# frozenreboot/rplidar_ros2_driver

Measured on AMD Instinct MI355X. Metric: Mpoints/s raw-scan->filtered PointCloud2, higher is better.
Workload: dtype u32/f32

## Files before the change

rplidar_ros2_driver_amd/csrc/rpl_device.hpp:

```cpp
#pragma once
#include <hip/hip_runtime.h>
#include <stdint.h>

#include "rplgpu.h"

namespace rpl {

constexpr int kBlock = 1024;
constexpr int kWaves = kBlock / 64;
constexpr int kIters = 32;
constexpr uint32_t kMaxN = 32768;
constexpr int kChunks = kIters * kWaves;
constexpr double kTwoPi = 6.283185307179586476925286766559;

struct Tables {
  const float *angle;
  const float *angle_inv;
  const float2 *cs;
  const float2 *cs_inv;
  const double *rcp;
  uint32_t *work_ctr;
  uint32_t n_cu;
  void *voxel_store;
  uint32_t voxel_store_wgs;
  uint32_t voxel_store_recs;
  unsigned long long *voxel_stats;
  unsigned long long *voxel_stats_host;
  int32_t voxel_split;
  const float *scan_t0;
  uint32_t *redo;
};

struct KParams {
  int32_t is_new_protocol;
  int32_t inverted;
  int32_t scan_processing;
  int32_t clip_enable;
  uint32_t q_min;
  float range_min;
  float range_max;
  float voxel_leaf;
  float ror_r2;
  uint32_t ror_k;
  double vox_scale;
  float vox_scale_f;
  int32_t vox_L;
  int32_t vox_bias;
  float inv_leaf;
  float leaf_s;
  float inv_leaf_s;
  uint32_t d_lo;
  uint32_t d_span;
  int32_t cell_range_safe;
  unsigned long long *dbg;
  uint32_t *cell_keys;
  int32_t fast_div;
  int32_t fast_d4000;
};

__device__ __forceinline__ uint32_t nd_q14(uint2 v) { return v.x & 0xFFFFu; }
// ... 114 lines not shown
```

rplidar_ros2_driver_amd/csrc/rpl_launch.hpp:

```cpp
#pragma once
#include <hip/hip_runtime.h>
#include <stdint.h>

#include "rplgpu.h"
#include "rplgpu_msg.h"
#include "rplgpu_comm.h"
#include "rpl_device.hpp"
#include "rpl_msg.hpp"

namespace rplmsg {
struct Prefix;
}

namespace rpl {

constexpr uint32_t kAscendUnsorted = 0x80000000u;
constexpr uint32_t kRorListedBit = 0x80000000u;
constexpr uint32_t kScanStatusBits =
    RPLGPU_SCAN_ALL_INVALID | RPLGPU_SCAN_CELL_RANGE | RPLGPU_SCAN_TABLE_FULL | RPLGPU_SCAN_OUT_TRUNCATED;
static_assert((kAscendUnsorted & kScanStatusBits) == 0, "internal ascend bit overlaps RPLGPU_SCAN_*");
static_assert((kRorListedBit & kScanStatusBits) == 0, "internal cloud bit overlaps RPLGPU_SCAN_*");
hipError_t launch_ascend(hipStream_t s, void *nodes, uint32_t n_stride, const uint32_t *n_per_scan,
                         uint32_t B, uint32_t *status, uint32_t *need_sort, bool defer_sort = false,
                         uint32_t *sort_stat = nullptr);
// ... 13 lines not shown
                              const Tables &T, const float *inc_table, const float *rinc_table,
                              bool fast, float *ranges, float *intens, uint32_t *beam_count,
                              uint32_t n_given = 0xFFFFFFFFu, const LsMsgOut *msg_out = nullptr);
hipError_t launch_validate_idx(hipStream_t s, const Tables &T, const float *inc_table,
                               const float *rinc_table, uint32_t max_count,
                               uint32_t *d_mismatches);
hipError_t launch_laserscan_raw(hipStream_t s, const void *nodes, uint32_t n_stride,
                                const uint32_t *n_per_scan, uint32_t B, const KParams &p,
                                float *ranges, float *intens, uint32_t *beam_count);
hipError_t launch_cloud(hipStream_t s, const void *nodes, uint32_t n_stride,
                        const uint32_t *n_per_scan, uint32_t B, const KParams &p, const Tables &T,
                        const uint32_t *keepmask, uint32_t mask_stride, float *xyzi,
                        uint32_t out_stride, uint32_t *n_points, uint32_t *status,
                        const float *motion = nullptr);
enum class ArenaForm : int { kXyzi = 0, kXyi = 1, kCells = 2 };
enum class RorMode : int { kNone = 0, kInside = 1, kListed = 2 };
struct VoxelLaunch {
  const void *nodes = nullptr;
  uint32_t n_stride = 0;
  const uint32_t *n_per_scan = nullptr;
  uint32_t B = 0;
  uint32_t group = 1;
  const float *motion = nullptr, *pose2d = nullptr;
  const uint32_t *keepmask = nullptr;
  uint32_t mask_stride = 0;
  RorMode ror = RorMode::kNone;
  float *xyzi = nullptr;
  uint32_t out_stride = 0;
  float *arena = nullptr;
  uint64_t arena_capacity = 0;
  uint64_t *arena_cursor = nullptr, *scan_start = nullptr;
  ArenaForm form = ArenaForm::kXyzi;
  uint32_t *n_points = nullptr, *status = nullptr;
};
hipError_t launch_cloud_voxel(hipStream_t s, const VoxelLaunch &v, const KParams &p, const Tables &T);
uint32_t voxel_max_workgroups(uint32_t n_cu);
inline uint64_t voxel_store_need(uint32_t group, uint32_t n_stride) {
  const uint64_t s = n_stride < kMaxN ? n_stride : kMaxN;
  return (uint64_t)(group ? group : 1u) * (s + 2u * ((s + 123u) / 124u) + 1u + 528u);
}
hipError_t launch_ror_mask(hipStream_t s, const void *nodes, uint32_t n_stride,
                           const uint32_t *n_per_scan, uint32_t B, const KParams &p,
                           const Tables &T, uint32_t *mask, uint32_t mask_stride,
                           bool listed = false, uint32_t group = 1);
hipError_t launch_validate_div(hipStream_t s, float d, float rd, uint32_t e_lo, uint32_t e_hi,
                               uint32_t *d_mismatches);
hipError_t launch_pack(hipStream_t s, const float *xyzi, uint32_t out_stride,
                       const uint32_t *n_points, uint32_t B, float *packed, uint64_t *offsets);

hipError_t launch_laserscan_to_cloud(hipStream_t s, const float *ranges, const float *intens,
                                     uint32_t n_stride, const uint32_t *beam_count, uint32_t B,
                                     const KParams &p, float *xyzi, uint32_t out_stride,
                                     uint32_t *n_points, uint32_t *status);

hipError_t launch_signal(hipStream_t s, uint32_t *flag, uint32_t seq);
hipError_t launch_stage_in(hipStream_t s, const void *src, void *dst, uint32_t n_words2);
hipError_t launch_pack_meta(hipStream_t s, const unsigned long long *cursor,
                            const unsigned long long *scan_start, const uint32_t *n_points,
                            uint32_t B, unsigned long long slot_points, uint32_t max_scans,
                            uint32_t *meta);
hipError_t launch_unpack_gathered(hipStream_t s, const float *points_all,
                                  unsigned long long slot_points, const uint32_t *meta_all,
                                  uint32_t meta_words, uint32_t world, uint32_t max_scans,
                                  float *packed, unsigned long long *total,
                                  unsigned long long *scan_start_all, uint32_t *n_points_all,
                                  uint32_t *status, uint32_t n_cu, bool xyi = false);
// ... 193 lines not shown
```

rplidar_ros2_driver_amd/csrc/rpl_voxel.hip:

```cpp
#include <algorithm>
#include <cstdlib>
#include <type_traits>

#include "rpl_device.hpp"
#include "rpl_launch.hpp"
#include "rpl_xf.hpp"

namespace rpl {

#ifndef RPL_VOXEL_THREADS
#define RPL_VOXEL_THREADS 1024
#endif
#ifndef RPL_VOXEL_WGS_PER_CU
#define RPL_VOXEL_WGS_PER_CU (RPL_VOXEL_THREADS == 512 ? 2 : 1)
#endif
constexpr int kVB = RPL_VOXEL_THREADS;
constexpr int kVW = kVB / 64;
constexpr int kVWG = RPL_VOXEL_WGS_PER_CU;
constexpr uint32_t kRecCap = kVWG == 2 ? 4096u : 7168u;
constexpr uint32_t kRecPerThread = kRecCap / kVB;
constexpr uint32_t kRowCap = kVWG == 2 ? 1024u : 2u * kVB;
constexpr uint32_t kRowsPerThread = kRowCap / kVB;
constexpr uint32_t kBucketCap = kRecCap + 3u * kRowCap;
constexpr uint32_t kEmptyKey = 0xFFFFFFFFu;
// ... 262 lines not shown
  return false;
}

template <int NS>
__device__ __forceinline__ void voxel_block_split(QueueSink &S,
                                                  const bool (&ok)[NS], const uint32_t (&key)[NS],
                                                  const uint32_t (&qx)[NS], const uint32_t (&qy)[NS],
                                                  const uint32_t (&ci)[NS]) {
#pragma unroll
  for (uint32_t cls = 0; cls < 2u; ++cls) {
    bool okc[NS];
    uint32_t keyc[NS], qxc[NS], qyc[NS], cic[NS];
#pragma unroll
    for (int j = 0; j < NS; ++j) {
      okc[j] = ok[j] && (((key[j] >> 16) ^ key[j]) & 1u) == cls;
      keyc[j] = key[j];
      qxc[j] = okc[j] ? qx[j] : 0u;
      qyc[j] = okc[j] ? qy[j] : 0u;
      cic[j] = okc[j] ? ci[j] : 0u;
    }
    voxel_block_pass<true, NS, kPassPlain>(S, okc, keyc, qxc, qyc, cic);
  }
}

__device__ __forceinline__ double run_sum_f64(uint32_t u) {
  double s = (double)u;
  if (u >= 0xF0000000u) s -= 4294967296.0;
  return s;
}

struct VoxelArena {
  float4 *base;
  unsigned long long *cursor;
  unsigned long long capacity;
  unsigned long long *scan_start;
  int xyi;
};
enum : int { kEmitLegacy = 0, kEmitArenaFirst = 1, kEmitCountOnly = 2, kEmitArenaKnown = 3, kEmitArenaTemp = 4 };

template <bool DBG>
struct PhaseClock {
  unsigned long long acc[8] = {0, 0, 0, 0, 0, 0, 0, 0}, mark = 0;
  __device__ __forceinline__ void start() {
    if (DBG) mark = clock64();
  }
  __device__ __forceinline__ void lap(int i) {
    if (DBG) {
      const unsigned long long now = clock64();
      acc[i] += now - mark;
      mark = now;
    }
  }
};

template <bool DBG, bool CELLS>
__device__ __forceinline__ uint32_t voxel_reduce(VoxelLds &L, const KParams &p,
                                                 float4 *__restrict__ out, uint32_t out_stride,
                                                 uint32_t b, uint32_t *ncell_out, int mode,
                                                 const VoxelArena &arena, bool normalised,
                                                 const float4 *out_buffer) {
  PhaseClock<DBG> pc;
  pc.start();
  auto flush_dbg = [&]() {
    if (DBG && p.dbg && threadIdx.x == 0) {
#pragma unroll
      for (int i = 1; i < 8; ++i) atomicAdd(&p.dbg[16 * b + i], pc.acc[i]);
// ... 511 lines not shown
                                                      unsigned long long *dbg_slot,
                                                      RorSide *rs = nullptr, uint32_t oob_off = 0u) {
  if constexpr (RORM == 1) {
    if (use_xf)
      voxel_stream<FAST_DIV, SAFE, SPLIT, false, true, false, true, AHEAD, true>(
          sink, p, cs, rsrc, blk0, blk_end, nullptr, 0u, sd.xf, q_min16, ibfe_off, ibfe_w, flags, nullptr, rs, oob_off);
    else if (q_min16)
      voxel_stream<FAST_DIV, SAFE, SPLIT, false, true, false, false, AHEAD, true>(
          sink, p, cs, rsrc, blk0, blk_end, nullptr, 0u, sd.xf, q_min16, ibfe_off, ibfe_w, flags, nullptr, rs, oob_off);
    else
      voxel_stream<FAST_DIV, SAFE, SPLIT, false, false, false, false, AHEAD, true>(
          sink, p, cs, rsrc, blk0, blk_end, nullptr, 0u, sd.xf, q_min16, ibfe_off, ibfe_w, flags, nullptr, rs, oob_off);
    return;
  }
#define RPL_VS(HQ, HM, XFB)                                                                         \
  voxel_stream<FAST_DIV, SAFE, SPLIT, DBG, HQ, HM, XFB, AHEAD>(sink, p, cs, rsrc, blk0, blk_end, \
                                                                     sd.ror_bits, mask_stride, sd.xf, \
                                                                     q_min16, ibfe_off, ibfe_w, flags, \
                                                                     dbg_slot)
  if constexpr (RORM == 2) {
    if (use_xf) RPL_VS(true, true, true);
    else RPL_VS(true, true, false);
    return;
  }
  if (use_xf) {
    if (sd.ror_bits) RPL_VS(true, true, true);
    else RPL_VS(true, false, true);
  } else if (sd.ror_bits) RPL_VS(true, true, false);
  else if (q_min16) RPL_VS(true, false, false);
  else RPL_VS(false, false, false);
#undef RPL_VS
}

template <bool DBG, int RORM = 0, bool CELLS = false, class FirstBand>
__device__ __forceinline__ void voxel_work_loop(VoxelLds &L, const KParams &p, const Tables &T,
                                                uint4 *__restrict__ G, float4 *__restrict__ xyzi,
                                                uint32_t out_stride, uint32_t *__restrict__ n_points,
                                                uint32_t *__restrict__ status, uint32_t B,
                                                uint32_t item0, const VoxelArena &arena,
                                                FirstBand &&first_band) {
  if (threadIdx.x < 256) L.rcp[threadIdx.x] = T.rcp[threadIdx.x];
  if constexpr (RORM == 2) B = min(B, (uint32_t)__builtin_amdgcn_readfirstlane((int)T.redo[0]));
  for (uint32_t bl = blockIdx.x; bl < B;) {
  const uint32_t b = RORM == 2 ? T.redo[4u + bl] : item0 + bl;
  bool abandoned = false;
  float4 *out = arena.base ? arena.base : xyzi + (size_t)b * out_stride;
  int emit_mode = arena.base ? kEmitArenaFirst : kEmitLegacy;
  unsigned long long arena_at = 0ull;

  if (threadIdx.x < 16) L.misc[threadIdx.x] = 0u;
  if (threadIdx.x == 0) {
    L.band_lo[0] = 0u;
    L.band_hi[0] = 0xFFFFFFFEu;
    L.misc[3] = 1u;
    L.tmp[28] = 0u;
    L.tmp[29] = 0u;
  }
  __syncthreads();

  uint32_t flags = 0;
  PhaseClock<DBG> pc;
  pc.start();

  bool first = true;
  bool leave_single_band_mode_early = false;
  bool from_store = false;
// ... 294 lines not shown
        float *dst = reinterpret_cast<float *>(arena.base) + 3u * (size_t)arena_at;
        for (uint32_t i = threadIdx.x; i < ncopy; i += kVB) {
          const float4 v = src[i];
          dst[3u * i] = v.x;
          dst[3u * i + 1u] = v.y;
          dst[3u * i + 2u] = v.w;
        }
      } else {
        float4 *dst = arena.base + arena_at;
        for (uint32_t i = threadIdx.x; i < ncopy; i += kVB) dst[i] = src[i];
      }
    }
  }
  if (DBG && p.dbg && threadIdx.x == 0) {
    atomicAdd(&p.dbg[16 * b], pc.acc[0]);
    atomicAdd(&p.dbg[16 * b + 2], pc.acc[2]);
  }

  if (flags) atomicOr(&L.misc[1], flags);
  __syncthreads();
  if (threadIdx.x == 0 && !abandoned) {
    const uint32_t total = L.misc[7];
    if (arena.base) {
      const unsigned long long room = arena_at >= arena.capacity ? 0ull : arena.capacity - arena_at;
      const uint32_t kept = (uint32_t)min((unsigned long long)total, room);
      arena.scan_start[b] = arena_at;
      n_points[b] = kept;
      if (status) status[b] = L.misc[1] | (kept < total ? RPLGPU_SCAN_OUT_TRUNCATED : 0u);
    } else {
      n_points[b] = min(total, out_stride);
      if (status) status[b] = L.misc[1] | ((total > out_stride) ? RPLGPU_SCAN_OUT_TRUNCATED : 0u);
    }
  }
  if (RORM != 2 && B <= gridDim.x) return;
  if (threadIdx.x == 0) L.tmp[31] = gridDim.x + atomicAdd(&T.work_ctr[0], 1u);
  __syncthreads();
  bl = L.tmp[31];
  __syncthreads();
  }
}

template <bool FAST_DIV, bool SAFE, bool DBG, bool SPLIT, int RORM = 0>
__global__ __launch_bounds__(kVB) __attribute__((amdgpu_waves_per_eu(kVB * kVWG / 256, kVB * kVWG / 256))) void k_cloud_voxel(
    const uint2 *__restrict__ nodes, uint32_t n_stride, const uint32_t *__restrict__ n_per_scan,
    KParams p, Tables T, const uint32_t *__restrict__ keepmask, uint32_t mask_stride,
    float4 *__restrict__ xyzi, uint32_t out_stride, uint32_t *__restrict__ n_points,
    uint32_t *__restrict__ status, uint32_t B, VoxelArena arena, uint4 *__restrict__ store,
    uint32_t group, uint32_t n_scans, const float *__restrict__ motion,
    const float *__restrict__ pose2d) {
  __shared__ VoxelLds L;
  uint4 *G = store + (size_t)blockIdx.x * 2u * T.voxel_store_recs;
  const float2 *cs = p.inverted ? T.cs_inv : T.cs;
  const uint32_t ishift = p.is_new_protocol ? 0u : 2u;
  const uint32_t ibfe_off = 16u + ishift, ibfe_w = 0xFFu >> ishift;
  const uint32_t q_min16 = p.clip_enable ? (min(p.q_min, 256u) << 16) : 0u;
  const bool use_xf = (group > 1u) || motion || pose2d;
  __shared__ RorSide Rs;
  auto phase_s = [&](uint32_t b, uint32_t, uint32_t &flags) -> bool {
    QueueSink sink{L, G};
    const uint32_t s_lo = b * group, s_hi = min(n_scans, s_lo + group);
    for (uint32_t sc = s_lo; sc < s_hi; ++sc) {
      const uint32_t n = (uint32_t)__builtin_amdgcn_readfirstlane(
          (int)min(n_per_scan[sc], min(n_stride, kMaxN)));
      const uint2 *scan = nodes + (size_t)sc * n_stride;
      const __amdgpu_buffer_rsrc_t scan_rsrc =
          __builtin_amdgcn_make_buffer_rsrc((void *)scan, 0, (int)(n * 8u), 0x00020000);
      const ScanSide sd = scan_side(sc, keepmask, mask_stride, motion, pose2d, T.scan_t0);
      const uint32_t blk0 = (uint32_t)__builtin_amdgcn_readfirstlane((int)wave_id());
      if constexpr (RORM == 1) {
        if (threadIdx.x == 0) { Rs.n_todo = 0u; Rs.n_todo2 = 0u; }
        __syncthreads();
        voxel_stream_dispatch<FAST_DIV, SAFE, SPLIT, false, RPL_VOXEL_AHEAD, 1>(
// ... 38 lines not shown
    bad += (div_by(0.0f, d, rd) != 0.0f);
    bad += (div_by(-0.0f, d, rd) != 0.0f);
  }
  if (bad) atomicAdd(mismatches, bad);
}

hipError_t launch_validate_div(hipStream_t s, float d, float rd, uint32_t e_lo, uint32_t e_hi,
                               uint32_t *d_mismatches) {
  hipLaunchKernelGGL(k_validate_div, dim3(256 * 16), dim3(256), 0, s, d, rd, e_lo, e_hi,
                     d_mismatches);
  return hipGetLastError();
}

uint32_t voxel_max_workgroups(uint32_t n_cu) { return (uint32_t)kVWG * (n_cu ? n_cu : 256u); }


hipError_t launch_cloud_voxel(hipStream_t s, const VoxelLaunch &v, const KParams &p, const Tables &T) {
  static_assert(sizeof(unsigned long long) == sizeof(uint64_t), "64-bit cursor");
  uint32_t B = v.B, group = v.group;
  const bool ror = v.ror != RorMode::kNone, listed = v.ror == RorMode::kListed;
  if (B == 0) return hipSuccess;
  if (ror && (!p.fast_div || !T.redo || p.dbg)) return hipErrorInvalidValue;
  if (listed && !v.keepmask) return hipErrorInvalidValue;
  if (v.form == ArenaForm::kCells && !ror && (p.dbg || !T.voxel_split)) return hipErrorInvalidValue;
  if (group == 0) group = 1;
  group = std::min(group, B);
  const uint32_t n_scans = B;
  B = (B + group - 1u) / group;
  if (!T.voxel_store || T.voxel_store_wgs == 0) return hipErrorInvalidValue;
  if (voxel_store_need(group, v.n_stride) > T.voxel_store_recs) return hipErrorInvalidValue;
  VoxelArena ar;
  ar.base = (float4 *)v.arena;
  ar.cursor = reinterpret_cast<unsigned long long *>(v.arena_cursor);
  ar.capacity = v.arena_capacity;
  ar.scan_start = reinterpret_cast<unsigned long long *>(v.scan_start);
  ar.xyi = v.arena ? (int)v.form : 0;
  if (kVWG == 2 && group > 1) return hipErrorInvalidValue;
  uint32_t grid = std::min<uint32_t>(std::min<uint32_t>(B, voxel_max_workgroups(T.n_cu)),
                                     T.voxel_store_wgs);
  if (const char *e = std::getenv("RPLGPU_VOXEL_GRID")) {
    const long g = std::atol(e);
    if (g > 0) grid = std::min<uint32_t>(grid, (uint32_t)g);
  }
  const bool with_stats = T.voxel_stats && T.voxel_stats_host && B >= 64u && !listed;
  Tables Tk = T;
  if (!with_stats) Tk.voxel_stats = nullptr;
  if (with_stats)
    if (hipError_t e = hipMemsetAsync(T.voxel_stats, 0, 16, s); e != hipSuccess) return e;
  if (grid < B || listed)
    if (hipError_t e = hipMemsetAsync(T.work_ctr, 0, 4, s); e != hipSuccess) return e;
#define RPL_LAUNCH_VOXEL(FD, SF, DB, SP)                                                          \
  hipLaunchKernelGGL((k_cloud_voxel<FD, SF, DB, SP>), dim3(grid), dim3(kVB), 0, s, (const uint2 *)v.nodes, \
                     v.n_stride, v.n_per_scan, p, Tk, v.keepmask, v.mask_stride, (float4 *)v.xyzi, v.out_stride, \
                     v.n_points, v.status, B, ar, (uint4 *)T.voxel_store, group, n_scans, v.motion, v.pose2d)
#define RPL_LAUNCH_VOXEL_SF(FD, DB, SP)                                                           \
  do {                                                                                             \
    if (p.cell_range_safe) RPL_LAUNCH_VOXEL(FD, true, DB, SP); else RPL_LAUNCH_VOXEL(FD, false, DB, SP); \
  } while (0)
#define RPL_LAUNCH_VOXEL_ROR(SF, SP, RM)                                                          \
  hipLaunchKernelGGL((k_cloud_voxel<true, SF, false, SP, RM>), dim3(grid), dim3(kVB), 0, s,         \
                     (const uint2 *)v.nodes, v.n_stride, v.n_per_scan, p, Tk, v.keepmask, v.mask_stride, \
                     (float4 *)v.xyzi, v.out_stride, v.n_points, v.status, B, ar, (uint4 *)T.voxel_store, \
                     group, n_scans, v.motion, v.pose2d)
#define RPL_LAUNCH_VOXEL_ROR_SF(SP, RM)                                                           \
  do {                                                                                             \
    if (p.cell_range_safe) RPL_LAUNCH_VOXEL_ROR(true, SP, RM); else RPL_LAUNCH_VOXEL_ROR(false, SP, RM); \
  } while (0)
  if (v.ror == RorMode::kInside) {
    if (T.voxel_split) RPL_LAUNCH_VOXEL_ROR_SF(true, 1); else RPL_LAUNCH_VOXEL_ROR_SF(false, 1);
  } else if (listed) {
    if (T.voxel_split) RPL_LAUNCH_VOXEL_ROR_SF(true, 2); else RPL_LAUNCH_VOXEL_ROR_SF(false, 2);
  } else
  if (p.dbg) {
    if (p.fast_div) RPL_LAUNCH_VOXEL_SF(true, true, false); else RPL_LAUNCH_VOXEL_SF(false, true, false);
  } else if (T.voxel_split) {
    if (p.fast_div) RPL_LAUNCH_VOXEL_SF(true, false, true); else RPL_LAUNCH_VOXEL_SF(false, false, true);
  } else {
    if (p.fast_div) RPL_LAUNCH_VOXEL_SF(true, false, false); else RPL_LAUNCH_VOXEL_SF(false, false, false);
  }
#undef RPL_LAUNCH_VOXEL_SF
#undef RPL_LAUNCH_VOXEL
#undef RPL_LAUNCH_VOXEL_ROR_SF
#undef RPL_LAUNCH_VOXEL_ROR
  if (with_stats) {
    if (hipError_t e = hipMemcpyAsync(T.voxel_stats_host, T.voxel_stats, 16, hipMemcpyDeviceToHost, s);
        e != hipSuccess)
      return e;
  }
  return hipGetLastError();
}

}
```

rplidar_ros2_driver_amd/csrc/rplgpu_api.hip:

```cpp
#include <hip/hip_runtime.h>
#include <dlfcn.h>

#include <algorithm>
#include <cmath>
#include <cstdio>
#include <cstdlib>
#include <cstring>
#include <limits>
#include <new>
#include <string>
#include <thread>
#include <vector>

#include "rplgpu.h"
#include "rplgpu_msg.h"
#include "rpl_launch.hpp"
#include "rpl_msg.hpp"
#include "rpl_comm_layout.hpp"
#include "rpl_cells.hpp"

struct VoxelBatchId {
  const void *nodes = nullptr;
  uint32_t n_stride = 0, B = 0, group = 0;
  bool operator==(const VoxelBatchId &o) const {
    return nodes == o.nodes && n_stride == o.n_stride && B == o.B && group == o.group;
  }
};

struct rplgpu_ctx {
  int device = -1;
  hipStream_t own_stream = nullptr;
  hipStream_t stream = nullptr;
  uint32_t max_n = 0, max_b = 0;
  float *d_angle = nullptr, *d_angle_inv = nullptr, *d_inc = nullptr, *d_rinc = nullptr;
  float2 *d_cs = nullptr, *d_cs_inv = nullptr;
  double *d_rcp = nullptr;
  unsigned char *h_pin = nullptr;
  unsigned char *d_pin = nullptr;
  bool zero_copy = true;
  bool spin_sync = true;
  size_t flag_off = 0;
  uint32_t scan_seq = 0;
  struct Pinned { unsigned char *host, *dev; size_t bytes; };
  std::vector<Pinned> pinned;
  unsigned char *d_nodes = nullptr, *d_out = nullptr;
  uint32_t *d_rormask = nullptr;
  uint32_t *d_redo = nullptr;
  int32_t ror_fused = 1;
  uint32_t *d_need_sort = nullptr;
  uint32_t need_sort_cap = 0;
  uint32_t *d_small = nullptr;
  bool div4000_ok = false;
  float leaf_checked = 0.0f;
  bool leaf_ok = false;
  bool idx_checked = false, idx_ok = false;
  uint32_t force_ieee = 0;
  unsigned long long *dbg = nullptr;
  uint32_t *cell_keys = nullptr;
  const float *scan_t0 = nullptr;
  unsigned long long *h_vstats = nullptr;
  uint32_t stats_group = 1;
  bool stats_valid = false;
  VoxelBatchId stats_id;
  struct VoxelDecision { VoxelBatchId id; bool split = false; bool valid = false; };
  VoxelDecision decisions[8];
  uint32_t next_decision = 0;
  int32_t last_split = 0;
  uint32_t n_cu = 0;
  void *d_vstore = nullptr;
  int32_t force_split = -1;
  bool dec_stage = true;
  uint32_t vstore_wgs = 0;
  uint32_t vstore_recs = 0;
  uint32_t *d_merge = nullptr;
  size_t merge_cap = 0;
  unsigned long long *d_mkeys = nullptr;
  size_t mkeys_cap = 0;
  bool mkeys_clean = true;
  float2 *d_medges = nullptr;
  size_t medges_cap = 0;
  bool mspec_valid = false;
  rplgpu_scan_merge_t mspec;
  rpl::MergeK mspec_k;
  unsigned char *d_dec = nullptr;
  size_t dec_cap = 0;
  unsigned char *d_scans = nullptr;
  size_t scans_cap = 0;
  uint32_t *d_dec_todo = nullptr;
  size_t dec_todo_cap = 0;
  bool check_ptrs = true;
  void *comm = nullptr;
  int32_t comm_rank = 0, comm_world = 0;
  hipStream_t xstream = nullptr;
// ... 112 lines not shown
    const uint32_t g = c->stats_group;
    if (items != 0 && entries <= items * g * 70000ull) {
      rplgpu_ctx::VoxelDecision *d = find(c->stats_id);
      if (!d) {
        d = &c->decisions[c->next_decision];
        c->next_decision = (c->next_decision + 1u) % (uint32_t)(sizeof(c->decisions) / sizeof(c->decisions[0]));
        d->id = c->stats_id;
        d->split = false;
        d->valid = true;
      }
      const unsigned long long avg = entries / (items * g);
      if (!d->split && avg > 6500ull) d->split = true;
      else if (d->split && avg < 4000ull) d->split = false;
    }
  }
  const rplgpu_ctx::VoxelDecision *mine = find(id);
  const bool split = mine ? mine->split : false;
  if (with_stats) {
    c->stats_id = id;
    c->stats_valid = true;
    c->stats_group = group;
  }
  c->last_split = (c->force_split >= 0 ? c->force_split != 0 : split) ? 1 : 0;
  return c->last_split != 0;
}

rpl::Tables tables_of(rplgpu_ctx *c) {
  rpl::Tables t;
  t.angle = c->d_angle;
  t.angle_inv = c->d_angle_inv;
  t.cs = c->d_cs;
  t.cs_inv = c->d_cs_inv;
  t.rcp = c->d_rcp;
  t.work_ctr = c->d_small + 16;
  t.n_cu = c->n_cu;
  t.voxel_store = c->d_vstore;
  t.voxel_store_wgs = c->vstore_wgs;
  t.voxel_store_recs = c->vstore_recs;
  t.voxel_stats = reinterpret_cast<unsigned long long *>(c->d_small + 24);
  t.voxel_stats_host = c->h_vstats;
  t.voxel_split = c->force_split > 0 ? 1 : 0;
  t.scan_t0 = c->scan_t0;
  t.redo = c->d_redo;
  return t;
}

void build_tables(std::vector<float> &angle, std::vector<float> &angle_inv,
                  std::vector<float2> &cs, std::vector<float2> &cs_inv, std::vector<float> &inc,
                  std::vector<float> &rinc) {
  angle.resize(65536);
  angle_inv.resize(65536);
  cs.resize(65536);
  cs_inv.resize(65536);
  for (int q = 0; q < 65536; ++q) {
    uint16_t angle_z_q14 = (uint16_t)q;
    float angle_deg = angle_z_q14 * 90.0f / 16384.0f;
    float angle_rad = angle_deg * (M_PI / 180.0f);
    if (angle_rad < 0.0f) angle_rad += 2.0f * M_PI;
    if (angle_rad >= 2.0f * M_PI) angle_rad -= 2.0f * M_PI;
    float inv = (2.0f * M_PI) - angle_rad;
    if (inv >= 2.0f * M_PI) inv -= 2.0f * M_PI;
    angle[q] = angle_rad;
    angle_inv[q] = inv;
    cs[q] = make_float2((float)std::cos((double)angle_rad), (float)std::sin((double)angle_rad));
    cs_inv[q] = make_float2((float)std::cos((double)inv), (float)std::sin((double)inv));
  }
  inc.resize(rpl::kMaxN + 1);
  inc[0] = 0.0f;
  for (uint32_t c = 1; c <= rpl::kMaxN; ++c)
    inc[c] = static_cast<float>((2.0 * M_PI) / static_cast<double>(c));
  rinc.resize(rpl::kMaxN + 1);
  rinc[0] = 0.0f;
  for (uint32_t c = 1; c <= rpl::kMaxN; ++c) rinc[c] = 1.0f / inc[c];
}

template <class T>
int32_t upload(rplgpu_ctx *c, T **dst, const std::vector<T> &src) {
  RPL_HIP(c, hipMalloc((void **)dst, src.size() * sizeof(T)));
  RPL_HIP(c, hipMemcpy(*dst, src.data(), src.size() * sizeof(T), hipMemcpyHostToDevice));
  return RPLGPU_OK;
}

void comm_teardown(rplgpu_ctx *c);

void free_ctx(rplgpu_ctx *c) {
  if (!c) return;
  if (c->device >= 0) (void)hipSetDevice(c->device);
  comm_teardown(c);
  if (c->d_angle) (void)hipFree(c->d_angle);
  if (c->d_angle_inv) (void)hipFree(c->d_angle_inv);
  if (c->d_inc) (void)hipFree(c->d_inc);
  if (c->d_rinc) (void)hipFree(c->d_rinc);
  if (c->d_cs) (void)hipFree(c->d_cs);
  if (c->d_cs_inv) (void)hipFree(c->d_cs_inv);
  if (c->d_rcp) (void)hipFree(c->d_rcp);
  if (c->d_nodes) (void)hipFree(c->d_nodes);
  if (c->d_out) (void)hipFree(c->d_out);
  if (c->d_small) (void)hipFree(c->d_small);
  if (c->d_rormask) (void)hipFree(c->d_rormask);
  if (c->d_redo) (void)hipFree(c->d_redo);
  if (c->d_need_sort) (void)hipFree(c->d_need_sort);
  if (c->d_dec) (void)hipFree(c->d_dec);
  if (c->d_scans) (void)hipFree(c->d_scans);
  if (c->d_dec_todo) (void)hipFree(c->d_dec_todo);
  if (c->d_vstore) (void)hipFree(c->d_vstore);
  if (c->d_merge) (void)hipFree(c->d_merge);
  if (c->d_mkeys) (void)hipFree(c->d_mkeys);
  if (c->d_medges) (void)hipFree(c->d_medges);
  if (c->h_vstats) (void)hipHostFree(c->h_vstats);
  if (c->h_pin) (void)hipHostFree(c->h_pin);
  if (c->own_stream) (void)hipStreamDestroy(c->own_stream);
  delete c;
}

bool device_readable(rplgpu_ctx *c, const void *ptr, const char *what) {
  if (!c->check_ptrs) return true;
  hipPointerAttribute_t a;
  std::memset(&a, 0, sizeof(a));
  const hipError_t e = hipPointerGetAttributes(&a, ptr);
  if (e != hipSuccess) {
    (void)hipGetLastError();
    c->err = std::string(what) + " is not device-accessible memory";
    return false;
  }
  if (a.type == hipMemoryTypeDevice && a.device != c->device) {
    int can = 0;
    if (hipDeviceCanAccessPeer(&can, c->device, a.device) != hipSuccess || !can) {
      c->err = std::string(what) + " lives on another device without peer access";
      return false;
    }
  }
// ... 189 lines not shown
  auto fail = [&](int32_t code) {
    g_create_err = c->err;
    free_ctx(c);
    return code;
  };
  if (hipStreamCreateWithFlags(&c->own_stream, hipStreamNonBlocking) != hipSuccess)
    return fail(RPLGPU_ERR_HIP);
  c->stream = c->own_stream;

  std::vector<float> angle, angle_inv, inc, rinc;
  std::vector<float2> cs, cs_inv;
  build_tables(angle, angle_inv, cs, cs_inv, inc, rinc);
  for (int q = 1; q < 65536; ++q) {
    if (!(angle[q] > angle[q - 1])) {
      c->err = "angle table not strictly increasing";
      return fail(RPLGPU_ERR_INVALID_ARG);
    }
  }
  std::vector<double> rcp(rpl::kMaxN + 1);
  rcp[0] = 0.0;
  for (uint32_t k = 1; k <= rpl::kMaxN; ++k) rcp[k] = 1.0 / static_cast<double>(k);
  int32_t rc;
  if ((rc = upload(c, &c->d_rcp, rcp)) || (rc = upload(c, &c->d_angle, angle)) || (rc = upload(c, &c->d_angle_inv, angle_inv)) ||
      (rc = upload(c, &c->d_cs, cs)) || (rc = upload(c, &c->d_cs_inv, cs_inv)) ||
      (rc = upload(c, &c->d_inc, inc)) || (rc = upload(c, &c->d_rinc, rinc)))
    return fail(rc);

  const size_t n = c->max_n;
  c->flag_off = stage_flag_off(n);
  if (hipHostMalloc((void **)&c->h_pin, stage_bytes(n), hipHostMallocDefault) != hipSuccess ||
      hipMalloc((void **)&c->d_nodes, n * 8 + kTail) != hipSuccess ||
      hipMalloc((void **)&c->d_out, n * 16 + kTail) != hipSuccess ||
      hipMalloc((void **)&c->d_small, 128) != hipSuccess ||
      hipMalloc((void **)&c->d_need_sort, ((size_t)c->max_b + 1u) * 4u) != hipSuccess ||
      hipMalloc((void **)&c->d_rormask, (size_t)c->max_b * kMaskStride * 4u) != hipSuccess ||
      hipMalloc((void **)&c->d_redo, ((size_t)c->max_b + 4u) * 4u) != hipSuccess) {
    c->err = "staging allocation failed";
    return fail(RPLGPU_ERR_HIP);
  }
  c->need_sort_cap = c->max_b;
  if (hipMemset(c->d_need_sort, 0, 4) != hipSuccess || hipMemset(c->d_redo, 0, 4) != hipSuccess) {
    c->err = "staging allocation failed";
    return fail(RPLGPU_ERR_HIP);
  }
  c->vstore_wgs = std::min<uint32_t>(c->max_b, rpl::voxel_max_workgroups(c->n_cu));
  c->vstore_recs = (uint32_t)rpl::voxel_store_need(1u, rpl::kMaxN);
  if (hipMalloc(&c->d_vstore, (size_t)c->vstore_wgs * c->vstore_recs * 32u) != hipSuccess) {
    c->err = "record store allocation failed";
    return fail(RPLGPU_ERR_HIP);
  }
  if (hipHostMalloc((void **)&c->h_vstats, 16, hipHostMallocDefault) == hipSuccess) {
    c->h_vstats[0] = c->h_vstats[1] = 0ull;
  } else {
    c->h_vstats = nullptr;
    (void)hipGetLastError();
  }
  if (hipHostGetDevicePointer((void **)&c->d_pin, c->h_pin, 0) != hipSuccess) c->d_pin = nullptr;
  if (const char *e = std::getenv("RPLGPU_ZERO_COPY")) c->zero_copy = std::atoi(e) != 0;
  if (!c->d_pin) c->zero_copy = false;
  if (const char *e = std::getenv("RPLGPU_SPIN_SYNC")) c->spin_sync = std::atoi(e) != 0;
  if (const char *e = std::getenv("RPLGPU_DEC_STAGE")) c->dec_stage = std::atoi(e) != 0;
  if (const char *e = std::getenv("RPLGPU_VOXEL_SPLIT")) c->force_split = std::atoi(e) != 0;
  if (const char *e = std::getenv("RPLGPU_ROR_FUSED")) c->ror_fused = std::atoi(e) != 0;
  std::memset(c->h_pin + c->flag_off, 0, kTail);
  if (hipMemset(c->d_small, 0, 128) != hipSuccess) {
    c->err = "staging clear failed";
    return fail(RPLGPU_ERR_HIP);
  }
  if (validate_divisor(c, 4000.0f, 127, 159, &c->div4000_ok) != RPLGPU_OK) return fail(RPLGPU_ERR_HIP);
  if (validate_divisor(c, 0.05f, 27, 167, &c->leaf_ok) != RPLGPU_OK) return fail(RPLGPU_ERR_HIP);
  c->leaf_checked = 0.05f;
  *out = c;
  return RPLGPU_OK;
}

int32_t rplgpu_destroy(rplgpu_handle_t h) {
  if (!h) return RPLGPU_ERR_INVALID_ARG;
  (void)hipSetDevice(h->device);
  (void)hipStreamSynchronize(h->stream);
  free_ctx(h);
  return RPLGPU_OK;
}

const char *rplgpu_last_error(rplgpu_handle_t h) {
  if (!h) return g_create_err.c_str();
  return h->err.c_str();
}

int32_t rplgpu_set_stream(rplgpu_handle_t h, void *hip_stream) {
  if (!h) return RPLGPU_ERR_INVALID_ARG;
  hipStream_t next = hip_stream ? (hipStream_t)hip_stream : h->own_stream;
  if (next != h->stream) {
    RPL_HIP(h, hipSetDevice(h->device));
    RPL_HIP(h, hipStreamSynchronize(h->stream));
  }
  h->stream = next;
  return RPLGPU_OK;
}

int32_t rplgpu_set_cell_key_output(rplgpu_handle_t h, uint32_t *d_cell_keys) {
  if (!h) return RPLGPU_ERR_INVALID_ARG;
  if (d_cell_keys && !device_readable(h, d_cell_keys, "d_cell_keys")) return RPLGPU_ERR_INVALID_ARG;
  h->cell_keys = d_cell_keys;
  return RPLGPU_OK;
}

int32_t rplgpu_set_scan_time_offsets_dev(rplgpu_handle_t h, const float *d_t0) {
  if (!h) return RPLGPU_ERR_INVALID_ARG;
  if (d_t0 && !device_readable(h, d_t0, "d_t0")) return RPLGPU_ERR_INVALID_ARG;
  h->scan_t0 = d_t0;
  return RPLGPU_OK;
}

int32_t rplgpu_set_voxel_aggregation(rplgpu_handle_t h, int32_t mode) {
  if (!h || mode < RPLGPU_VOXEL_AGG_AUTO || mode > RPLGPU_VOXEL_AGG_TWO_CLASS) return RPLGPU_ERR_INVALID_ARG;
  h->force_split = mode == RPLGPU_VOXEL_AGG_AUTO ? -1 : (mode == RPLGPU_VOXEL_AGG_TWO_CLASS ? 1 : 0);
  return RPLGPU_OK;
}

int32_t rplgpu_debug_set_cycle_buffer(rplgpu_handle_t h, void *d_buf) {
  if (!h) return RPLGPU_ERR_INVALID_ARG;
  h->dbg = (unsigned long long *)d_buf;
  return RPLGPU_OK;
}
int32_t rplgpu_debug_ascend_sorted(rplgpu_handle_t h, uint32_t *count) {
  if (!h || !count) return RPLGPU_ERR_INVALID_ARG;
  RPL_HIP(h, hipSetDevice(h->device));
  RPL_HIP(h, hipStreamSynchronize(h->stream));
  RPL_HIP(h, hipMemcpy(count, h->d_small + 28, 4, hipMemcpyDeviceToHost));
// ... 118 lines not shown
  plan->kp = to_kparams(*p);
  rpl::KParams &kp = plan->kp;
  if (p->voxel_enable) {
    if (h->leaf_checked != p->voxel_leaf) {
      int32_t vrc = validate_divisor(h, p->voxel_leaf, 27, 167, &h->leaf_ok);
      if (vrc) return vrc;
      h->leaf_checked = p->voxel_leaf;
    }
    kp.fast_div = (use_fast_d4000(h) && use_fast_leaf(h)) ? 1 : 0;
  }
  kp.fast_d4000 = use_fast_d4000(h) ? 1 : 0;
  kp.dbg = h->dbg;
  kp.cell_keys = h->cell_keys;
  plan->T = tables_of(h);
  if (p->ror_enable) {
    plan->ror_inside = ror_runs_inside(h, req, *p, kp);
    if (!plan->ror_inside) {
      RPL_HIP(h, rpl::launch_ror_mask(h->stream, d_nodes, n_stride, d_n_per_scan, B, kp, plan->T,
                                      h->d_rormask, kMaskStride));
      plan->mask = h->d_rormask;
    }
  }
  if (req.cells) {
    kp.cell_keys = nullptr;
    kp.dbg = nullptr;
  }
  if (p->voxel_enable) {
    plan->T.voxel_split = voxel_split_for(h, d_nodes, n_stride, B, req.group) ? 1 : 0;
    if (req.cells && !plan->ror_inside) plan->T.voxel_split = 1;
  }
  return RPLGPU_OK;
}

static int32_t run_voxel(rplgpu_handle_t h, const CloudPlan &plan, rpl::VoxelLaunch v,
                         bool defer_listed = false) {
  if (v.arena) RPL_HIP(h, hipMemsetAsync(v.arena_cursor, 0, 8, h->stream));
  v.keepmask = plan.mask;
  v.mask_stride = kMaskStride;
  if (plan.ror_inside) {
    RPL_HIP(h, hipMemsetAsync(h->d_redo, 0, 4, h->stream));
    v.ror = rpl::RorMode::kInside;
  }
  RPL_HIP(h, rpl::launch_cloud_voxel(h->stream, v, plan.kp, plan.T));
  if (!plan.ror_inside || defer_listed) return RPLGPU_OK;
  RPL_HIP(h, rpl::launch_ror_mask(h->stream, v.nodes, v.n_stride, v.n_per_scan, v.B, plan.kp, plan.T,
                                  h->d_rormask, kMaskStride, true, std::max(1u, std::min(v.group, v.B))));
  v.keepmask = h->d_rormask;
  v.ror = rpl::RorMode::kListed;
  RPL_HIP(h, rpl::launch_cloud_voxel(h->stream, v, plan.kp, plan.T));
  return RPLGPU_OK;
}

static int32_t cloud_arena_impl(rplgpu_handle_t h, const rplgpu_node_t *d_nodes, uint32_t n_stride,
                               const uint32_t *d_n_per_scan, uint32_t B, const rplgpu_params_t *p,
                               float *d_arena, uint64_t arena_capacity, uint64_t *d_cursor,
                               uint64_t *d_scan_start, uint32_t *d_n_points, uint32_t *d_status,
                               bool xyi) {
  int32_t rc = check_batch(h, d_nodes, n_stride, d_n_per_scan, B);
  if (rc) return rc;
  if (!p || !d_arena || !d_cursor || !d_scan_start || !d_n_points) return RPLGPU_ERR_INVALID_ARG;
  if (!p->voxel_enable) {
    h->err = "rplgpu_cloud_arena_dev needs voxel_enable";
    return RPLGPU_ERR_INVALID_ARG;
  }
  CloudPlan plan;
  if ((rc = prepare_cloud(h, d_nodes, n_stride, d_n_per_scan, B, p, CloudRequest{}, &plan))) return rc;
  rpl::VoxelLaunch v{d_nodes, n_stride, d_n_per_scan, B};
  v.arena = d_arena;
  v.arena_capacity = arena_capacity;
  v.arena_cursor = d_cursor;
  v.scan_start = d_scan_start;
  v.form = xyi ? rpl::ArenaForm::kXyi : rpl::ArenaForm::kXyzi;
  v.n_points = d_n_points;
  v.status = d_status;
  return run_voxel(h, plan, v);
}

int32_t rplgpu_cloud_arena_dev(rplgpu_handle_t h, const rplgpu_node_t *d_nodes, uint32_t n_stride,
                               const uint32_t *d_n_per_scan, uint32_t B, const rplgpu_params_t *p,
                               float *d_arena, uint64_t arena_capacity, uint64_t *d_cursor,
                               uint64_t *d_scan_start, uint32_t *d_n_points, uint32_t *d_status) {
  return cloud_arena_impl(h, d_nodes, n_stride, d_n_per_scan, B, p, d_arena, arena_capacity, d_cursor,
                          d_scan_start, d_n_points, d_status, false);
// ... 3022 lines not shown
```

Baseline: 290,700.

## Fold voxel arena cursor/stat resets into kernel via last-arriver workgroup

For arena voxel launches without inside-ROR, the per-call memsets of the arena cursor, stats and work counter and the stats D2H memcpy are replaced by a persistent device word block. The last workgroup to finish, detected with an atomic counter, publishes the cursor and stats (stats go straight to pinned host memory) and resets the counters for the next call. The aim is to cut each call down to one GPU command and so remove launch and queue overhead. It adds a grid-wide atomic and fence at kernel end, plus dirty-state tracking that must stay correct across stream switches and errors.

```diff
diff --git a/rplidar_ros2_driver_amd/csrc/rpl_device.hpp b/rplidar_ros2_driver_amd/csrc/rpl_device.hpp
--- a/rplidar_ros2_driver_amd/csrc/rpl_device.hpp
+++ b/rplidar_ros2_driver_amd/csrc/rpl_device.hpp
@@ -19,6 +19,7 @@
   const float2 *cs;
   const float2 *cs_inv;
   const double *rcp;
+  uint32_t *voxel_words;
   uint32_t *work_ctr;
   uint32_t n_cu;
   void *voxel_store;
@@ -26,6 +27,7 @@
   uint32_t voxel_store_recs;
   unsigned long long *voxel_stats;
   unsigned long long *voxel_stats_host;
+  unsigned long long *voxel_stats_pub;
   int32_t voxel_split;
   const float *scan_t0;
   uint32_t *redo;
diff --git a/rplidar_ros2_driver_amd/csrc/rpl_launch.hpp b/rplidar_ros2_driver_amd/csrc/rpl_launch.hpp
--- a/rplidar_ros2_driver_amd/csrc/rpl_launch.hpp
+++ b/rplidar_ros2_driver_amd/csrc/rpl_launch.hpp
@@ -69,6 +69,7 @@
   uint64_t *arena_cursor = nullptr, *scan_start = nullptr;
   ArenaForm form = ArenaForm::kXyzi;
   uint32_t *n_points = nullptr, *status = nullptr;
+  bool one_command = false;
 };
 hipError_t launch_cloud_voxel(hipStream_t s, const VoxelLaunch &v, const KParams &p, const Tables &T);
 uint32_t voxel_max_workgroups(uint32_t n_cu);
diff --git a/rplidar_ros2_driver_amd/csrc/rpl_voxel.hip b/rplidar_ros2_driver_amd/csrc/rpl_voxel.hip
--- a/rplidar_ros2_driver_amd/csrc/rpl_voxel.hip
+++ b/rplidar_ros2_driver_amd/csrc/rpl_voxel.hip
@@ -318,6 +318,7 @@
 struct VoxelArena {
   float4 *base;
   unsigned long long *cursor;
+  unsigned long long *cursor_out;
   unsigned long long capacity;
   unsigned long long *scan_start;
   int xyi;
@@ -895,6 +896,26 @@
 #undef RPL_VS
 }
 
+__device__ __forceinline__ void voxel_last_arriver(const Tables &T, const VoxelArena &arena) {
+  if (!arena.cursor_out || threadIdx.x != 0) return;
+  uint32_t *done = T.voxel_words + 7;
+  __builtin_amdgcn_fence(__ATOMIC_RELEASE, "agent");
+  asm volatile("s_waitcnt vmcnt(0) lgkmcnt(0)" ::: "memory");
+  const uint32_t before_me = __hip_atomic_fetch_add(done, 1u, __ATOMIC_RELAXED, __HIP_MEMORY_SCOPE_AGENT);
+  if (before_me != gridDim.x - 1u) return;
+  *arena.cursor_out = __hip_atomic_exchange(arena.cursor, 0ull, __ATOMIC_RELAXED, __HIP_MEMORY_SCOPE_AGENT);
+  if (T.voxel_stats) {
+    const unsigned long long entries =
+        __hip_atomic_exchange(&T.voxel_stats[0], 0ull, __ATOMIC_RELAXED, __HIP_MEMORY_SCOPE_AGENT);
+    const unsigned long long items =
+        __hip_atomic_exchange(&T.voxel_stats[1], 0ull, __ATOMIC_RELAXED, __HIP_MEMORY_SCOPE_AGENT);
+    __hip_atomic_store(&T.voxel_stats_pub[0], entries, __ATOMIC_RELAXED, __HIP_MEMORY_SCOPE_SYSTEM);
+    __hip_atomic_store(&T.voxel_stats_pub[1], items, __ATOMIC_RELAXED, __HIP_MEMORY_SCOPE_SYSTEM);
+  }
+  __hip_atomic_store(T.work_ctr, 0u, __ATOMIC_RELAXED, __HIP_MEMORY_SCOPE_AGENT);
+  __hip_atomic_store(done, 0u, __ATOMIC_RELAXED, __HIP_MEMORY_SCOPE_AGENT);
+}
+
 template <bool DBG, int RORM = 0, bool CELLS = false, class FirstBand>
 __device__ __forceinline__ void voxel_work_loop(VoxelLds &L, const KParams &p, const Tables &T,
                                                 uint4 *__restrict__ G, float4 *__restrict__ xyzi,
@@ -1255,12 +1276,13 @@
       if (status) status[b] = L.misc[1] | ((total > out_stride) ? RPLGPU_SCAN_OUT_TRUNCATED : 0u);
     }
   }
-  if (RORM != 2 && B <= gridDim.x) return;
+  if (RORM != 2 && B <= gridDim.x) break;
   if (threadIdx.x == 0) L.tmp[31] = gridDim.x + atomicAdd(&T.work_ctr[0], 1u);
   __syncthreads();
   bl = L.tmp[31];
   __syncthreads();
   }
+  if constexpr (RORM == 0) voxel_last_arriver(T, arena);
 }
 
 template <bool FAST_DIV, bool SAFE, bool DBG, bool SPLIT, int RORM = 0>
@@ -1365,6 +1387,13 @@
   VoxelArena ar;
   ar.base = (float4 *)v.arena;
   ar.cursor = reinterpret_cast<unsigned long long *>(v.arena_cursor);
+  ar.cursor_out = nullptr;
+  const bool one_command = v.one_command;
+  if (one_command) {
+    if (!v.arena || !v.arena_cursor || !T.voxel_words || ror) return hipErrorInvalidValue;
+    ar.cursor = reinterpret_cast<unsigned long long *>(T.voxel_words);
+    ar.cursor_out = reinterpret_cast<unsigned long long *>(v.arena_cursor);
+  }
   ar.capacity = v.arena_capacity;
   ar.scan_start = reinterpret_cast<unsigned long long *>(v.scan_start);
   ar.xyi = v.arena ? (int)v.form : 0;
@@ -1375,13 +1404,14 @@
     const long g = std::atol(e);
     if (g > 0) grid = std::min<uint32_t>(grid, (uint32_t)g);
   }
-  const bool with_stats = T.voxel_stats && T.voxel_stats_host && B >= 64u && !listed;
+  const bool with_stats = T.voxel_stats && T.voxel_stats_host && B >= 64u && !listed &&
+                          (!one_command || T.voxel_stats_pub);
   Tables Tk = T;
   if (!with_stats) Tk.voxel_stats = nullptr;
-  if (with_stats)
-    if (hipError_t e = hipMemsetAsync(T.voxel_stats, 0, 16, s); e != hipSuccess) return e;
-  if (grid < B || listed)
-    if (hipError_t e = hipMemsetAsync(T.work_ctr, 0, 4, s); e != hipSuccess) return e;
+  if (!one_command && (with_stats || grid < B || listed)) {
+    if (!T.voxel_words) return hipErrorInvalidValue;
+    if (hipError_t e = hipMemsetAsync(T.voxel_words, 0, 32, s); e != hipSuccess) return e;
+  }
 #define RPL_LAUNCH_VOXEL(FD, SF, DB, SP)                                                          \
   hipLaunchKernelGGL((k_cloud_voxel<FD, SF, DB, SP>), dim3(grid), dim3(kVB), 0, s, (const uint2 *)v.nodes, \
                      v.n_stride, v.n_per_scan, p, Tk, v.keepmask, v.mask_stride, (float4 *)v.xyzi, v.out_stride, \
@@ -1415,7 +1445,7 @@
 #undef RPL_LAUNCH_VOXEL
 #undef RPL_LAUNCH_VOXEL_ROR_SF
 #undef RPL_LAUNCH_VOXEL_ROR
-  if (with_stats) {
+  if (with_stats && !one_command) {
     if (hipError_t e = hipMemcpyAsync(T.voxel_stats_host, T.voxel_stats, 16, hipMemcpyDeviceToHost, s);
         e != hipSuccess)
       return e;
diff --git a/rplidar_ros2_driver_amd/csrc/rplgpu_api.hip b/rplidar_ros2_driver_amd/csrc/rplgpu_api.hip
--- a/rplidar_ros2_driver_amd/csrc/rplgpu_api.hip
+++ b/rplidar_ros2_driver_amd/csrc/rplgpu_api.hip
@@ -50,6 +50,8 @@
   uint32_t *d_need_sort = nullptr;
   uint32_t need_sort_cap = 0;
   uint32_t *d_small = nullptr;
+  uint32_t *d_vwords = nullptr;
+  bool voxel_words_dirty = true;
   bool div4000_ok = false;
   float leaf_checked = 0.0f;
   bool leaf_ok = false;
@@ -59,6 +61,7 @@
   uint32_t *cell_keys = nullptr;
   const float *scan_t0 = nullptr;
   unsigned long long *h_vstats = nullptr;
+  unsigned long long *d_vstats = nullptr;
   uint32_t stats_group = 1;
   bool stats_valid = false;
   VoxelBatchId stats_id;
@@ -237,13 +240,15 @@
   t.cs = c->d_cs;
   t.cs_inv = c->d_cs_inv;
   t.rcp = c->d_rcp;
-  t.work_ctr = c->d_small + 16;
+  t.voxel_words = c->d_vwords;
+  t.work_ctr = c->d_vwords + 6;
   t.n_cu = c->n_cu;
   t.voxel_store = c->d_vstore;
   t.voxel_store_wgs = c->vstore_wgs;
   t.voxel_store_recs = c->vstore_recs;
-  t.voxel_stats = reinterpret_cast<unsigned long long *>(c->d_small + 24);
+  t.voxel_stats = reinterpret_cast<unsigned long long *>(c->d_vwords + 2);
   t.voxel_stats_host = c->h_vstats;
+  t.voxel_stats_pub = c->d_vstats;
   t.voxel_split = c->force_split > 0 ? 1 : 0;
   t.scan_t0 = c->scan_t0;
   t.redo = c->d_redo;
@@ -302,6 +307,7 @@
   if (c->d_nodes) (void)hipFree(c->d_nodes);
   if (c->d_out) (void)hipFree(c->d_out);
   if (c->d_small) (void)hipFree(c->d_small);
+  if (c->d_vwords) (void)hipFree(c->d_vwords);
   if (c->d_rormask) (void)hipFree(c->d_rormask);
   if (c->d_redo) (void)hipFree(c->d_redo);
   if (c->d_need_sort) (void)hipFree(c->d_need_sort);
@@ -557,6 +563,7 @@
       hipMalloc((void **)&c->d_nodes, n * 8 + kTail) != hipSuccess ||
       hipMalloc((void **)&c->d_out, n * 16 + kTail) != hipSuccess ||
       hipMalloc((void **)&c->d_small, 128) != hipSuccess ||
+      hipMalloc((void **)&c->d_vwords, 64) != hipSuccess ||
       hipMalloc((void **)&c->d_need_sort, ((size_t)c->max_b + 1u) * 4u) != hipSuccess ||
       hipMalloc((void **)&c->d_rormask, (size_t)c->max_b * kMaskStride * 4u) != hipSuccess ||
       hipMalloc((void **)&c->d_redo, ((size_t)c->max_b + 4u) * 4u) != hipSuccess) {
@@ -574,10 +581,12 @@
     c->err = "record store allocation failed";
     return fail(RPLGPU_ERR_HIP);
   }
-  if (hipHostMalloc((void **)&c->h_vstats, 16, hipHostMallocDefault) == hipSuccess) {
+  if (hipHostMalloc((void **)&c->h_vstats, 16, hipHostMallocDefault) == hipSuccess &&
+      hipHostGetDevicePointer((void **)&c->d_vstats, c->h_vstats, 0) == hipSuccess) {
     c->h_vstats[0] = c->h_vstats[1] = 0ull;
   } else {
-    c->h_vstats = nullptr;
+    if (c->h_vstats) (void)hipHostFree(c->h_vstats);
+    c->h_vstats = c->d_vstats = nullptr;
     (void)hipGetLastError();
   }
   if (hipHostGetDevicePointer((void **)&c->d_pin, c->h_pin, 0) != hipSuccess) c->d_pin = nullptr;
@@ -588,7 +597,7 @@
   if (const char *e = std::getenv("RPLGPU_VOXEL_SPLIT")) c->force_split = std::atoi(e) != 0;
   if (const char *e = std::getenv("RPLGPU_ROR_FUSED")) c->ror_fused = std::atoi(e) != 0;
   std::memset(c->h_pin + c->flag_off, 0, kTail);
-  if (hipMemset(c->d_small, 0, 128) != hipSuccess) {
+  if (hipMemset(c->d_small, 0, 128) != hipSuccess || hipMemset(c->d_vwords, 0, 64) != hipSuccess) {
     c->err = "staging clear failed";
     return fail(RPLGPU_ERR_HIP);
   }
@@ -620,6 +629,7 @@
     RPL_HIP(h, hipStreamSynchronize(h->stream));
   }
   h->stream = next;
+  h->voxel_words_dirty = true;
   return RPLGPU_OK;
 }
 
@@ -804,9 +814,16 @@
   return RPLGPU_OK;
 }
 
-static int32_t run_voxel(rplgpu_handle_t h, const CloudPlan &plan, rpl::VoxelLaunch v,
-                         bool defer_listed = false) {
-  if (v.arena) RPL_HIP(h, hipMemsetAsync(v.arena_cursor, 0, 8, h->stream));
+static int32_t run_voxel_commands(rplgpu_handle_t h, const CloudPlan &plan, rpl::VoxelLaunch v,
+                                  bool defer_listed) {
+  v.one_command = v.arena && v.B != 0 && !plan.ror_inside;
+  if (v.one_command) {
+    if (h->voxel_words_dirty) RPL_HIP(h, hipMemsetAsync(h->d_vwords, 0, 32, h->stream));
+    h->voxel_words_dirty = false;
+  } else {
+    if (v.B != 0) h->voxel_words_dirty = true;
+    if (v.arena) RPL_HIP(h, hipMemsetAsync(v.arena_cursor, 0, 8, h->stream));
+  }
   v.keepmask = plan.mask;
   v.mask_stride = kMaskStride;
   if (plan.ror_inside) {
@@ -821,6 +838,13 @@
   v.ror = rpl::RorMode::kListed;
   RPL_HIP(h, rpl::launch_cloud_voxel(h->stream, v, plan.kp, plan.T));
   return RPLGPU_OK;
+}
+
+static int32_t run_voxel(rplgpu_handle_t h, const CloudPlan &plan, const rpl::VoxelLaunch &v,
+                         bool defer_listed = false) {
+  const int32_t rc = run_voxel_commands(h, plan, v, defer_listed);
+  if (rc) h->voxel_words_dirty = true;
+  return rc;
 }
 
 static int32_t cloud_arena_impl(rplgpu_handle_t h, const rplgpu_node_t *d_nodes, uint32_t n_stride,
```

Measured after the change: 292,800, median of 6. About the same (+0.7%).
